# multimodallearning/convexAdam

Hardware: AMD Instinct MI355X
Metric: volume-pairs/sec (160x192x224 MIND convex+Adam(80it)) (higher is better)
Workload: dtype f32

## Files before the change

### convexadam_amd/csrc/certify.hip

```cpp
#include <hip/hip_runtime.h>
#include <stdlib.h>

#include "cvx_common.h"

namespace cvx {

#define CERT_CLO ((float)((1.0 - 1.0 / 65536.0) / 729.0))
#define CERT_CHI ((float)((1.0 + 1.0 / 65536.0) / 729.0))
#define CERT_TINY 1.0e-40f
__device__ __forceinline__ float cert_lower(float s) { return fmaxf(__builtin_fmaf(s, CERT_CLO, -CERT_TINY), 0.0f); }
__device__ __forceinline__ float cert_upper(float s) { return __builtin_fmaf(s, CERT_CHI, fminf(s, CERT_TINY)); }

__device__ __forceinline__ unsigned ordered_bits(float v) {
    unsigned b = __float_as_uint(v);
    b = (b & 0x80000000u) ? ~b : (b | 0x80000000u);
    if (v != v) b = 0u;
    return b;
}
__device__ __forceinline__ float from_ordered_bits(unsigned b) { return __uint_as_float((b & 0x80000000u) ? (b & 0x7fffffffu) : ~b); }

struct CertRec { unsigned x, box; int kp; float bound, slo, uc, ub, ua; };

struct CertProb {
    const float* ssdu; const float* fix; const float* mov; const float* tail;
    unsigned long long* key; unsigned* sec;
    int* idx0; int* idxA; int* idxB;
    float* smin;
    unsigned* list; int* counts;
    unsigned long long* work; unsigned work_cap;
    struct CertRec* rec;
    float* u;
    int64_t* argmin_out;
};
struct CertGeo { int C, h, w, d, hw, n, K, ntail; long long tail_from; };
struct CertArgs { CertProb p[2]; CertGeo g; const float* mesh; float coef; int pass; };

template <bool WAVE>
__device__ __forceinline__ void cert_sync() {
    if (WAVE) { __builtin_amdgcn_fence(__ATOMIC_RELEASE, "wavefront"); __builtin_amdgcn_s_waitcnt(0xC07F); __builtin_amdgcn_wave_barrier(); __builtin_amdgcn_fence(__ATOMIC_ACQUIRE, "wavefront"); }
    else __syncthreads();
}
template <bool WAVE>
__device__ float cert_exact_entry_t(const CertGeo& G, const CertProb& P, int k, int xlin, float* sm, int lane) {
    const int n = G.n, nn = n * n, h = G.h, w = G.w, d = G.d, hw = G.hw;
    const int iH = k % n, iW = (k / n) % n, iD = k / nn;
    const int x = xlin % d, y = (xlin / d) % w, z = xlin / (d * w);
    const size_t v = (size_t)h * w * d;
    for (int t = lane; t < 125; t += 64) {
        const int a = t / 25 - 2, b = (t / 5) % 5 - 2, c = t % 5 - 2;
        const int pz = z + a, py = y + b, px = x + c;
        float val = 0.0f;
        if (pz >= 0 && pz < h && py >= 0 && py < w && px >= 0 && px < d) {
            const long long flat = (((long long)pz * nn + iW * n + iD) * w + py) * d + px;
            if (G.ntail > 0 && flat >= G.tail_from) val = P.tail[iH * 32 + (int)(flat - G.tail_from)];
            else {
                const int mz = pz + iH - hw, my = py + iW - hw, mx = px + iD - hw;
                const bool inb = mz >= 0 && mz < h && my >= 0 && my < w && mx >= 0 && mx < d;
                const float* fp = P.fix + ((size_t)pz * w + py) * d + px;
                const float* mp = P.mov + ((size_t)(inb ? mz : 0) * w + (inb ? my : 0)) * d + (inb ? mx : 0);
                float a0 = 0.0f, a1 = 0.0f;
                for (int c0 = 0; c0 < G.C; c0 += 16) {
                    float fv[16], mv[16];
#pragma unroll
                    for (int i = 0; i < 16; ++i) {
                        const bool on = c0 + i < G.C;
                        fv[i] = on ? fp[(size_t)(c0 + i) * v] : 0.0f;
                        mv[i] = (on && inb) ? mp[(size_t)(c0 + i) * v] : 0.0f;
                    }
#pragma unroll
                    for (int i = 0; i < 16; ++i) {
                        if (c0 + i < G.C) {
                            const float df = fv[i] - mv[i];
                            a0 += df * df;
                        }
                    }
                    if (c0 + 16 <= G.C) { a1 += a0; a0 = 0.0f; }
                }
                val = G.C >= 16 ? a0 + a1 : a0;
            }
        }
        sm[t] = val;
    }
    cert_sync<WAVE>();
    if (lane < 27) {
        const int a = lane / 9 - 1, b = (lane / 3) % 3 - 1, c = lane % 3 - 1;
        const int pz = z + a, py = y + b, px = x + c;
        float s = 0.0f;
        const bool in = pz >= 0 && pz < h && py >= 0 && py < w && px >= 0 && px < d;
        if (in) {
            for (int aa = -1; aa <= 1; ++aa)
                for (int bb = -1; bb <= 1; ++bb)
                    for (int cc = -1; cc <= 1; ++cc) {
                        const int qz = pz + aa, qy = py + bb, qx = px + cc;
                        if (qz >= 0 && qz < h && qy >= 0 && qy < w && qx >= 0 && qx < d) s += sm[((a + aa + 2) * 5 + (b + bb + 2)) * 5 + (c + cc + 2)];
                    }
            s = div_exact<27>(s);
        }
        sm[128 + lane] = in ? s : -1.0f;
    }
    cert_sync<WAVE>();
    float s = 0.0f;
    for (int t = 0; t < 27; ++t) {
        const float b = sm[128 + t];
        if (b >= 0.0f || b != b) s += b;
    }
    cert_sync<WAVE>();
    return div_exact<27>(s);
}

__device__ float cert_exact_entry(const CertGeo& G, const CertProb& P, int k, int xlin, float* sm, int lane) { return cert_exact_entry_t<false>(G, P, k, xlin, sm, lane); }
__device__ float cert_exact_entry_wave(const CertGeo& G, const CertProb& P, int k, int xlin, float* sm, int lane) { return cert_exact_entry_t<true>(G, P, k, xlin, sm, lane); }

__global__ __launch_bounds__(256) void k_cert_plain_stream(CertArgs A, int kslice, int vec4) {
    const CertProb& P = A.p[blockIdx.z];
    const size_t v = (size_t)A.g.h * A.g.w * A.g.d;
    const int K = A.g.K;
    const size_t x0 = ((size_t)blockIdx.x * blockDim.x + threadIdx.x) * 4;
    const int k0 = blockIdx.y * kslice, k1 = min(k0 + kslice, K);
    if (x0 >= v) return;
    const int nv = (int)min((size_t)4, v - x0);
    const float INF = __uint_as_float(0x7f800000u);
    float best[4], second[4];
    int bi[4];
    bool tiny[4] = {false, false, false, false};
    const float* p = P.ssdu + (size_t)k0 * v + x0;
    auto load4 = [&](const float* q, float (&c4)[4]) {
        if (vec4) { const float4 t = *reinterpret_cast<const float4*>(q); c4[0] = t.x; c4[1] = t.y; c4[2] = t.z; c4[3] = t.w; }
        else {
#pragma unroll
            for (int j = 0; j < 4; ++j) c4[j] = j < nv ? q[j] : 0.0f;
        }
    };
    {
        float c4[4];
        load4(p, c4);
#pragma unroll
        for (int j = 0; j < 4; ++j) { best[j] = c4[j]; bi[j] = k0; second[j] = INF; tiny[j] = (c4[j] > 0.0f) & (c4[j] < 1.0e-36f); }
        p += v;
    }
#pragma unroll 8
    for (int k = k0 + 1; k < k1; ++k, p += v) {
        float c4[4];
        load4(p, c4);
#pragma unroll
        for (int j = 0; j < 4; ++j) {
            const float c = c4[j];
            tiny[j] = tiny[j] | ((c > 0.0f) & (c < 1.0e-36f));
            const bool lt = argmin_better(c, best[j]);
            second[j] = fminf(second[j], lt ? best[j] : c);
            best[j] = lt ? c : best[j];
            bi[j] = lt ? k : bi[j];
        }
    }
#pragma unroll
    for (int j = 0; j < 4; ++j) {
        if (j >= nv) continue;
        const unsigned long long mine = pack_min_key(best[j], (unsigned)bi[j]);
        const unsigned long long old = atomicMin(&P.key[x0 + j], mine);
        unsigned cand = second[j] == INF ? 0xffffffffu : ordered_bits(second[j]);
        if (old != ~0ull) {
            const unsigned loser = (unsigned)((old < mine ? mine : old) >> 32);
            cand = loser < cand ? loser : cand;
        }
        if (tiny[j]) cand = 0u;
        if (cand != 0xffffffffu) atomicMin(&P.sec[x0 + j], cand);
    }
}

__global__ __launch_bounds__(256) void k_cert_plain_finalize(CertArgs A) {
    const CertProb& P = A.p[blockIdx.y];
    const size_t v = (size_t)A.g.h * A.g.w * A.g.d;
    const size_t x = (size_t)blockIdx.x * blockDim.x + threadIdx.x;
    if (x >= v) return;
    const unsigned long long key = P.key[x];
    const unsigned b1 = (unsigned)(key >> 32), b2 = P.sec[x];
    const int k1 = (int)(unsigned)(key & 0xffffffffull);
    const float s1 = b1 == 0u ? __uint_as_float(0x7fc00000u) : from_ordered_bits(b1);
    P.smin[x] = s1;
    P.idx0[x] = k1;
    if (P.argmin_out) P.argmin_out[x] = k1;
    bool certain = b1 == 0u || b2 == 0xffffffffu;
    if (!certain && b2 != 0u) certain = s1 == 0.0f || cert_lower(from_ordered_bits(b2)) > cert_upper(s1);
    if (!certain) P.list[atomicAdd(&P.counts[0], 1)] = (unsigned)x;
}

__global__ __launch_bounds__(64) void k_cert_plain_resolve(CertArgs A) {
    __shared__ float sm[160];
    const CertProb& P = A.p[blockIdx.y];
    const size_t v = (size_t)A.g.h * A.g.w * A.g.d;
    const int K = A.g.K, lane = threadIdx.x;
    const int cnt = P.counts[0];
    for (int e = blockIdx.x; e < cnt; e += gridDim.x) {
        const unsigned x = P.list[e];
        const float* col = P.ssdu + x;
        const float U = cert_upper(P.smin[x]);
        unsigned long long bestkey = ~0ull;
        for (int kb = 0; kb < K; kb += 1024) {
            float s[16];
#pragma unroll
            for (int i = 0; i < 16; ++i) { const int k = kb + 64 * i + lane; s[i] = k < K ? col[(size_t)k * v] : __uint_as_float(0x7f800000u); }
#pragma unroll
            for (int i = 0; i < 16; ++i) {
                const unsigned long long mz = __ballot(s[i] == 0.0f);
                if (mz) {
                    const unsigned long long key = pack_min_key(0.0f, (unsigned)(kb + 64 * i + __ffsll((long long)mz) - 1));
                    bestkey = key < bestkey ? key : bestkey;
                }
                const bool mine = s[i] != 0.0f && cert_lower(s[i]) <= U;
                const unsigned long long m = __ballot(mine);
                if (m) {
                    const int nm = __popcll(m);
                    int base = 0;
                    if (lane == 0) base = atomicAdd(&P.counts[8], nm);
                    base = __shfl(base, 0);
                    const int slot = base + __popcll(m & ((1ull << lane) - 1ull));
                    if (mine && (unsigned)slot < P.work_cap) P.work[slot] = ((unsigned long long)x << 32) | (unsigned)(kb + 64 * i + lane);
                    unsigned long long rest = __ballot(mine && (unsigned)slot >= P.work_cap);
                    while (rest) {
                        const int l = __ffsll((long long)rest) - 1;
                        rest &= rest - 1;
                        const int kk = kb + 64 * i + l;
                        const float ex = cert_exact_entry(A.g, P, kk, (int)x, sm, lane);
                        const unsigned long long key = pack_min_key(ex, (unsigned)kk);
                        bestkey = key < bestkey ? key : bestkey;
                    }
                }
            }
        }
        if (lane == 0) P.key[x] = bestkey;
    }
}
__global__ __launch_bounds__(256) void k_cert_plain_eval(CertArgs A) {
    __shared__ float smem[4][160];
    const CertProb& P = A.p[blockIdx.y];
    const int lane = threadIdx.x & 63, wv = threadIdx.x >> 6;
    const int n = min(P.counts[8], (int)P.work_cap);
    for (int e = blockIdx.x * 4 + wv; e < n; e += gridDim.x * 4) {
        const unsigned long long it = P.work[e];
        const unsigned x = (unsigned)(it >> 32);
        const int kk = (int)(unsigned)(it & 0xffffffffull);
        const float ex = cert_exact_entry_wave(A.g, P, kk, (int)x, smem[wv], lane);
        if (lane == 0) atomicMin(&P.key[x], pack_min_key(ex, (unsigned)kk));
    }
}
__global__ __launch_bounds__(256) void k_cert_plain_commit(CertArgs A) {
    const CertProb& P = A.p[blockIdx.y];
    const int cnt = P.counts[0];
    for (int e = blockIdx.x * blockDim.x + threadIdx.x; e < cnt; e += gridDim.x * blockDim.x) {
        const unsigned x = P.list[e];
        const int kw = (int)(unsigned)(P.key[x] & 0xffffffffull);
        P.idx0[x] = kw;
        if (P.argmin_out) P.argmin_out[x] = kw;
    }
}

struct CertMesh {
    const float* ax;
    int n; float rn;
    __device__ __forceinline__ void split(int k, int& ic, int& ib, int& ia) const {
        const int q = (int)(((float)k + 0.5f) * rn);
        ic = k - q * n;
        ia = (int)(((float)q + 0.5f) * rn);
        ib = q - ia * n;
    }
};
__device__ __forceinline__ CertMesh cert_mesh_load(float* lds96, const float* __restrict__ mesh, int K, int n) {
    const int t = threadIdx.x;
    if (t < n) { lds96[t] = mesh[t]; lds96[32 + t] = mesh[K + t * n]; lds96[64 + t] = mesh[2 * K + t * n * n]; }
    __syncthreads();
    return CertMesh{lds96, n, 1.0f / (float)n};
}

__device__ __forceinline__ void cert_smooth_winner(const int* __restrict__ idx, const CertMesh& M, int h, int w, int d, size_t i,
                                                   float& o0, float& o1, float& o2) {
    const int x = (int)(i % d), y = (int)((i / d) % w), z = (int)(i / ((size_t)d * w));
    float s0 = 0.f, s1 = 0.f, s2 = 0.f;
#pragma unroll
    for (int a = -1; a <= 1; ++a) {
        const int za = z + a;
        const bool zok = za >= 0 && za < h;
        const int zc = zok ? za : z;
        int kk[9];
        bool ok[9];
#pragma unroll
        for (int b = -1; b <= 1; ++b)
#pragma unroll
            for (int c = -1; c <= 1; ++c) {
                const int yb = y + b, xc = x + c;
                const bool in = zok && yb >= 0 && yb < w && xc >= 0 && xc < d;
                const int t = (b + 1) * 3 + (c + 1);
                ok[t] = in;
                kk[t] = idx[((size_t)zc * w + (in ? yb : y)) * d + (in ? xc : x)];
            }
        float m0[9], m1[9], m2[9];
#pragma unroll
        for (int t = 0; t < 9; ++t) {
            int ic, ib, ia;
            M.split(kk[t], ic, ib, ia);
            m0[t] = M.ax[ic]; m1[t] = M.ax[32 + ib]; m2[t] = M.ax[64 + ia];
        }
#pragma unroll
        for (int t = 0; t < 9; ++t) {
            s0 += ok[t] ? m0[t] : 0.0f;
            s1 += ok[t] ? m1[t] : 0.0f;
            s2 += ok[t] ? m2[t] : 0.0f;
        }
    }
    o0 = fdiv(s0, 27.0f);
    o1 = fdiv(s1, 27.0f);
    o2 = fdiv(s2, 27.0f);
}

__device__ __forceinline__ float cert_pen(const CertMesh& M, int k, float uc, float ub, float ua, float coef) {
    int ic, ib, ia;
    M.split(k, ic, ib, ia);
    const float e0 = M.ax[ic] - uc, e1 = M.ax[32 + ib] - ub, e2 = M.ax[64 + ia] - ua;
    float q = e0 * e0;
    q += e1 * e1;
    q += e2 * e2;
    return coef * q;
}

struct CertBox {
    float uc, ub, ua, slo, bound;
    int c_lo, c_hi, b_lo, b_hi, a_lo, a_hi;
    long long vol;
    bool degenerate;
};
__device__ __forceinline__ CertBox cert_box(const CertMesh& M, float uc, float ub, float ua, float coef, int K, int n, int kp,
                                            float ssdu_kp, float smin_u, const float* __restrict__ col, size_t v, int refine_above) {
    CertBox c;
    c.uc = uc; c.ub = ub; c.ua = ua;
    c.slo = cert_lower(smin_u);
    c.bound = cert_upper(ssdu_kp) + cert_pen(M, kp, uc, ub, ua, coef);
    const float hwf = (float)((n - 1) / 2);
    auto close_box = [&]() {
        const float qmax = fdiv((c.bound - c.slo) + fabsf(c.bound) * 2.384185791015625e-07f, coef) * 1.00001f;
        const float R = fsqrt(fmaxf(qmax, 0.0f)) * 1.00001f + 1.0e-4f;
        c.c_lo = max((int)ceilf(c.uc - R + hwf), 0); c.c_hi = min((int)floorf(c.uc + R + hwf), n - 1);
        c.b_lo = max((int)ceilf(c.ub - R + hwf), 0); c.b_hi = min((int)floorf(c.ub + R + hwf), n - 1);
        c.a_lo = max((int)ceilf(c.ua - R + hwf), 0); c.a_hi = min((int)floorf(c.ua + R + hwf), n - 1);
        c.vol = (long long)max(c.c_hi - c.c_lo + 1, 0) * max(c.b_hi - c.b_lo + 1, 0) * max(c.a_hi - c.a_lo + 1, 0);
        c.degenerate = !(coef > 0.0f) || !(R == R) || c.vol <= 0;
    };
    close_box();
    if (!c.degenerate && c.vol > refine_above && uc == uc && ub == ub && ua == ua) {
        const int kn = (min(max((int)rintf(ua + hwf), 0), n - 1) * n + min(max((int)rintf(ub + hwf), 0), n - 1)) * n + min(max((int)rintf(uc + hwf), 0), n - 1);
        if (kn != kp) {
            const float near_hi = cert_upper(col[(size_t)kn * v]) + cert_pen(M, kn, uc, ub, ua, coef);
            if (near_hi < c.bound) { c.bound = near_hi; close_box(); }
        }
    }
    if (c.degenerate) { c.c_lo = c.b_lo = c.a_lo = 0; c.c_hi = c.b_hi = c.a_hi = n - 1; c.vol = (long long)n * n * n; }
    return c;
}

__global__ __launch_bounds__(64) void k_cert_voxel(CertArgs A, int refine) {
    const CertProb& P = A.p[blockIdx.y];
    const int h = A.g.h, w = A.g.w, d = A.g.d, K = A.g.K, n = A.g.n;
    const size_t v = (size_t)h * w * d;
    const size_t x = (size_t)blockIdx.x * blockDim.x + threadIdx.x;
    __shared__ float axes[96];
    const CertMesh M = cert_mesh_load(axes, A.mesh, K, n);
    if (x >= v) return;
    const int* prev = A.pass == 1 ? P.idx0 : ((A.pass & 1) ? P.idxB : P.idxA);
    int* next = (A.pass & 1) ? P.idxA : P.idxB;
    const int kp = prev[x];
    const float s_kp = P.ssdu[(size_t)kp * v + x];
    const float sm_x = P.smin[x];
    float uc, ub, ua;
    cert_smooth_winner(prev, M, h, w, d, x, uc, ub, ua);
    P.u[x] = uc; P.u[v + x] = ub; P.u[2 * v + x] = ua;
    if (sm_x != sm_x) { next[x] = P.idx0[x]; return; }
    const CertBox c = cert_box(M, uc, ub, ua, A.coef, K, n, kp, s_kp, sm_x, P.ssdu + x, v, refine);
    constexpr int NB = 8;
    const unsigned boxpack = (unsigned)c.c_lo | ((unsigned)c.c_hi << 5) | ((unsigned)c.b_lo << 10) | ((unsigned)c.b_hi << 15) | ((unsigned)c.a_lo << 20) | ((unsigned)c.a_hi << 25) | (c.degenerate ? 1u << 30 : 0u);
    const CertRec rec = {(unsigned)x, boxpack, kp, c.bound, c.slo, c.uc, c.ub, c.ua};
    if (c.vol > NB) { P.rec[atomicAdd(&P.counts[A.pass], 1)] = rec; return; }
    int kk[NB];
    float pen[NB], val[NB];
    bool need[NB];
    {
        int ic = c.c_lo, ib = c.b_lo, ia = c.a_lo;
#pragma unroll
        for (int j = 0; j < NB; ++j) {
            const bool in = j < (int)c.vol;
            kk[j] = (ia * n + ib) * n + ic;
            pen[j] = cert_pen(M, kk[j], c.uc, c.ub, c.ua, A.coef);
            need[j] = in && !(c.slo + pen[j] > c.bound);
            if (j + 1 < (int)c.vol) {
                if (++ic > c.c_hi) { ic = c.c_lo; if (++ib > c.b_hi) { ib = c.b_lo; ++ia; } }
            }
        }
    }
#pragma unroll
    for (int j = 0; j < NB; ++j) val[j] = need[j] ? P.ssdu[(size_t)kk[j] * v + x] : 0.0f;
    float lo1 = 0.f, lo2 = 0.f, U = __uint_as_float(0x7f800000u);
    int k1 = -1, cnt = 0;
#pragma unroll
    for (int j = 0; j < NB; ++j) {
        if (!need[j]) continue;
        const float lo = cert_lower(val[j]) + pen[j], hi = cert_upper(val[j]) + pen[j];
        U = fminf(U, hi);
        if (cnt == 0) { lo1 = lo; k1 = kk[j]; }
        else if (lo < lo1) { lo2 = lo1; lo1 = lo; k1 = kk[j]; }
        else if (cnt == 1 || lo < lo2) lo2 = lo;
        ++cnt;
    }
    if (cnt == 0) { next[x] = kp; return; }
    if (cnt == 1 || lo2 > U) { next[x] = k1; return; }
    P.rec[atomicAdd(&P.counts[A.pass], 1)] = rec;
}

__global__ __launch_bounds__(256) void k_cert_wave(CertArgs A) {
    __shared__ float smem[4][160];
    __shared__ float axes[96];
    const CertProb& P = A.p[blockIdx.y];
    const int h = A.g.h, w = A.g.w, d = A.g.d, K = A.g.K, n = A.g.n;
    const size_t v = (size_t)h * w * d;
    const int lane = threadIdx.x & 63, wv = threadIdx.x >> 6;
    float* sm = smem[wv];
    const CertMesh M = cert_mesh_load(axes, A.mesh, K, n);
    int* next = (A.pass & 1) ? P.idxA : P.idxB;
    const int cnt = P.counts[A.pass];
    const float INF = __uint_as_float(0x7f800000u);
    for (int e = blockIdx.x * 4 + wv; e < cnt; e += gridDim.x * 4) {
        const CertRec r = P.rec[e];
        const size_t x = r.x;
        const int kp = r.kp;
        const float* col = P.ssdu + x;
        CertBox c;
        c.uc = r.uc; c.ub = r.ub; c.ua = r.ua; c.slo = r.slo; c.bound = r.bound;
        c.c_lo = r.box & 31; c.c_hi = (r.box >> 5) & 31; c.b_lo = (r.box >> 10) & 31; c.b_hi = (r.box >> 15) & 31; c.a_lo = (r.box >> 20) & 31; c.a_hi = (r.box >> 25) & 31;
        c.degenerate = ((r.box >> 30) & 1u) != 0;
        c.vol = (long long)(c.c_hi - c.c_lo + 1) * (c.b_hi - c.b_lo + 1) * (c.a_hi - c.a_lo + 1);
        const int nc = c.c_hi - c.c_lo + 1, nb = c.b_hi - c.b_lo + 1, ncb = nc * nb;
        const float rc = 1.0f / (float)nc, rab = 1.0f / (float)ncb;
        unsigned long long key = ~0ull;
        float lo2 = INF, U = INF;
        constexpr int NL = 12;
        for (long long i0 = 0; i0 < c.vol; i0 += 64 * NL) {
            int kk[NL];
            float pen[NL], val[NL];
            bool need[NL];
#pragma unroll
            for (int j = 0; j < NL; ++j) {
                need[j] = false; kk[j] = 0; pen[j] = 0.0f;
                if (i0 + 64 * j < c.vol) {
                    const int i = (int)i0 + lane + 64 * j;
                    need[j] = i < (int)c.vol;
                    const int ii = need[j] ? i : 0;
                    const int qa = (int)(((float)ii + 0.5f) * rab), ra = ii - qa * ncb;
                    const int qb = (int)(((float)ra + 0.5f) * rc);
                    const int ic = c.c_lo + ra - qb * nc, ib = c.b_lo + qb, ia = c.a_lo + qa;
                    kk[j] = (ia * n + ib) * n + ic;
                    pen[j] = cert_pen(M, kk[j], c.uc, c.ub, c.ua, A.coef);
                    need[j] = need[j] && (c.degenerate || !(c.slo + pen[j] > c.bound));
                }
            }
#pragma unroll
            for (int j = 0; j < NL; ++j) val[j] = need[j] ? col[(size_t)kk[j] * v] : 0.0f;
#pragma unroll
            for (int j = 0; j < NL; ++j) {
                if (!need[j]) continue;
                const float lo = cert_lower(val[j]) + pen[j], hi = cert_upper(val[j]) + pen[j];
                U = fminf(U, hi);
                const unsigned long long kx = pack_min_key(lo, (unsigned)kk[j]);
                if (kx < key) { if (key != ~0ull) lo2 = fminf(lo2, from_ordered_bits((unsigned)(key >> 32))); key = kx; }
                else lo2 = fminf(lo2, lo);
            }
        }
        unsigned long long gkey = key;
        for (int o = 32; o > 0; o >>= 1) { const unsigned long long t = __shfl_xor(gkey, o); gkey = t < gkey ? t : gkey; }
        float mine2 = key == gkey ? lo2 : fminf(lo2, key != ~0ull ? from_ordered_bits((unsigned)(key >> 32)) : INF);
        for (int o = 32; o > 0; o >>= 1) { mine2 = fminf(mine2, __shfl_xor(mine2, o)); U = fminf(U, __shfl_xor(U, o)); }
        if (gkey == ~0ull) { if (lane == 0) next[x] = kp; continue; }
        if (mine2 > U) { if (lane == 0) next[x] = (int)(unsigned)(gkey & 0xffffffffull); continue; }
        if (lane == 0) atomicAdd(&P.counts[7], 1);
        unsigned long long bestkey = ~0ull;
        for (long long i0 = 0; i0 < c.vol; i0 += 64 * NL) {
            int kk[NL];
            float pen[NL], val[NL];
            bool need[NL];
#pragma unroll
            for (int j = 0; j < NL; ++j) {
                need[j] = false; kk[j] = 0; pen[j] = 0.0f;
                if (i0 + 64 * j < c.vol) {
                    const int i = (int)i0 + lane + 64 * j;
                    need[j] = i < (int)c.vol;
                    const int ii = need[j] ? i : 0;
                    const int qa = (int)(((float)ii + 0.5f) * rab), ra = ii - qa * ncb;
                    const int qb = (int)(((float)ra + 0.5f) * rc);
                    kk[j] = ((c.a_lo + qa) * n + c.b_lo + qb) * n + c.c_lo + ra - qb * nc;
                    pen[j] = cert_pen(M, kk[j], c.uc, c.ub, c.ua, A.coef);
                    need[j] = need[j] && (c.degenerate || !(c.slo + pen[j] > c.bound));
                }
            }
#pragma unroll
            for (int j = 0; j < NL; ++j) val[j] = need[j] ? col[(size_t)kk[j] * v] : 0.0f;
#pragma unroll
            for (int j = 0; j < NL; ++j) {
                if (!(i0 + 64 * j < c.vol)) continue;
                unsigned long long m = __ballot(need[j] && cert_lower(val[j]) + pen[j] <= U);
                while (m) {
                    const int l = __ffsll((long long)m) - 1;
                    m &= m - 1;
                    const int k2 = __shfl(kk[j], l);
                    const float sk = __shfl(val[j], l), pk = __shfl(pen[j], l);
                    const float ex = sk == 0.0f ? 0.0f : cert_exact_entry_wave(A.g, P, k2, (int)x, sm, lane);
                    const unsigned long long kx = pack_min_key(ex + pk, (unsigned)k2);
                    bestkey = kx < bestkey ? kx : bestkey;
                }
            }
        }
        if (lane == 0) next[x] = (int)(unsigned)(bestkey & 0xffffffffull);
    }
}

__global__ __launch_bounds__(256) void k_cert_gather(CertArgs A) {
    const CertProb& P = A.p[blockIdx.y];
    const size_t v = (size_t)A.g.h * A.g.w * A.g.d;
    const size_t i = (size_t)blockIdx.x * blockDim.x + threadIdx.x;
    __shared__ float axes[96];
    const CertMesh M = cert_mesh_load(axes, A.mesh, A.g.K, A.g.n);
    if (i >= v) return;
    const int* prev = A.pass == 1 ? P.idx0 : ((A.pass & 1) ? P.idxB : P.idxA);
    float o0, o1, o2;
    cert_smooth_winner(prev, M, A.g.h, A.g.w, A.g.d, i, o0, o1, o2);
    P.u[i] = o0; P.u[v + i] = o1; P.u[2 * v + i] = o2;
}

__global__ __launch_bounds__(256) void k_cert_arm(CertArgs A, int nprob) {
    const size_t v = (size_t)A.g.h * A.g.w * A.g.d;
    const size_t i = (size_t)blockIdx.x * blockDim.x + threadIdx.x;
    for (int q = 0; q < nprob; ++q) {
        if (i < v) { A.p[q].key[i] = ~0ull; A.p[q].sec[i] = 0xffffffffu; }
        if (i < 16) A.p[q].counts[i] = 0;
    }
}

void launch_corr_tail_compact(const float* fix, const float* mov, int C, int h, int w, int d, int hw, int sad, float* tail, hipStream_t s);

static size_t cert_work_cap(size_t v) { return 4 * v + 65536; }
struct CertCarve { unsigned long long* key; unsigned* sec; int* idx0; int* idxA; int* idxB; float* smin; unsigned* list; CertRec* rec; int* counts; float* tail; unsigned long long* work; unsigned work_cap; };
static CertCarve cert_layout(Carver& cv, int h, int w, int d, int hw, bool plain) {
    const size_t v = (size_t)h * w * d;
    const int n = 2 * hw + 1;
    CertCarve c{};
    c.key = cv.take<unsigned long long>(v);
    c.sec = cv.take<unsigned>(v);
    c.idx0 = cv.take<int>(v);
    c.smin = cv.take<float>(v);
    c.list = cv.take<unsigned>(v);
    c.counts = cv.take<int>(16);
    c.work_cap = (unsigned)cert_work_cap(v);
    c.work = cv.take<unsigned long long>(c.work_cap);
    c.tail = cv.take<float>((size_t)32 * n);
    if (!plain) {
        c.idxA = cv.take<int>(v); c.idxB = cv.take<int>(v);
        c.rec = cv.take<CertRec>(v);
    }
    return c;
}
size_t corr_certify_workspace_bytes(int, int h, int w, int d, int hw, bool plain) { Carver m; cert_layout(m, h, w, d, hw, plain); return ws_query(m); }
static CertGeo cert_geo(int C, int h, int w, int d, int hw) {
    CertGeo g;
    g.C = C; g.h = h; g.w = w; g.d = d; g.hw = hw; g.n = 2 * hw + 1; g.K = g.n * g.n * g.n;
    const long long ncols = (long long)h * g.n * g.n * w * d;
    g.tail_from = (ncols / 32) * 32;
    g.ntail = (int)(ncols - g.tail_from);
    return g;
}
static CertProb cert_prob(const float* ssdu, const float* fix, const float* mov, const CertCarve& c, float* u, int64_t* argmin_out) {
    return CertProb{ssdu, fix, mov, c.tail, c.key, c.sec, c.idx0, c.idxA, c.idxB, c.smin, c.list, c.counts, c.work, c.work_cap, c.rec, u, argmin_out};
}

static void cert_arm(CertArgs& A, int nprob, hipStream_t s) {
    const CertGeo& g = A.g;
    const size_t v = (size_t)g.h * g.w * g.d;
    hipLaunchKernelGGL(k_cert_arm, dim3((unsigned)cdiv64((int64_t)(v > 16 ? v : 16), 256)), dim3(256), 0, s, A, nprob);
    for (int q = 0; q < nprob; ++q)
        if (g.ntail > 0) launch_corr_tail_compact(A.p[q].fix, A.p[q].mov, g.C, g.h, g.w, g.d, g.hw, 0, const_cast<float*>(A.p[q].tail), s);
}
static void cert_stream(CertArgs A, int q0, int nq, hipStream_t s) {
    const CertGeo& g = A.g;
    const size_t v = (size_t)g.h * g.w * g.d;
    const int K = g.K;
    if (q0) { A.p[0] = A.p[q0]; }
    bool vec4 = v % 4 == 0;
    for (int q = 0; q < nq; ++q) vec4 = vec4 && (reinterpret_cast<uintptr_t>(A.p[q].ssdu) & 15) == 0;
    const int xb = (int)cdiv64((int64_t)cdiv64((int64_t)v, 4), 256);
    int nslices = cdiv(512, xb);
    if (nslices > K) nslices = K;
    if (nslices < 1) nslices = 1;
    const int kslice = cdiv(K, nslices);
    nslices = cdiv(K, kslice);
    hipLaunchKernelGGL(k_cert_plain_stream, dim3(xb, nslices, nq), dim3(256), 0, s, A, kslice, vec4 ? 1 : 0);
}
static int cert_finish(CertArgs& A, int nprob, hipStream_t s) {
    const size_t v = (size_t)A.g.h * A.g.w * A.g.d;
    hipLaunchKernelGGL(k_cert_plain_finalize, dim3((unsigned)cdiv64((int64_t)v, 256), nprob), dim3(256), 0, s, A);
    hipLaunchKernelGGL(k_cert_plain_resolve, dim3(256, nprob), dim3(64), 0, s, A);
    hipLaunchKernelGGL(k_cert_plain_eval, dim3(256, nprob), dim3(256), 0, s, A);
    hipLaunchKernelGGL(k_cert_plain_commit, dim3(8, nprob), dim3(256), 0, s, A);
    return check_last("certified argmin");
}
static int cert_plain(CertArgs& A, int nprob, bool arm, hipStream_t s) {
    if (arm) cert_arm(A, nprob, s);
    cert_stream(A, 0, nprob, s);
    return cert_finish(A, nprob, s);
}

int corr_certified_argmin(const float* ssdu, const float* fix, const float* mov, int C, int h, int w, int d, int hw, int64_t* argmin,
                          void* workspace, size_t workspace_bytes, hipStream_t s) {
    if (workspace_bytes < corr_certify_workspace_bytes(C, h, w, d, hw, true)) return fail(CVX_ERR_WORKSPACE, "certified argmin: workspace too small");
    Carver cv(workspace);
    const CertCarve c = cert_layout(cv, h, w, d, hw, true);
    CertArgs A{};
    A.g = cert_geo(C, h, w, d, hw);
    A.p[0] = cert_prob(ssdu, fix, mov, c, nullptr, argmin);
    A.p[1] = A.p[0];
    return cert_plain(A, 1, true, s);
}

int coupled_convex_cert_impl(const float* ssduA, const float* fixA, const float* movA, float* outA, void* wsA, const float* ssduB, const float* fixB,
                             const float* movB, float* outB, void* wsB, const float* mesh, int C, int h, int w, int d, int hw, size_t workspace_bytes,
                             hipStream_t s, int stage) {
    if (workspace_bytes < corr_certify_workspace_bytes(C, h, w, d, hw, false)) return fail(CVX_ERR_WORKSPACE, "certified coupled convex: workspace too small");
    const int nprob = ssduB ? 2 : 1;
    CertArgs A{};
    A.g = cert_geo(C, h, w, d, hw);
    A.mesh = mesh;
    Carver cva(wsA), cvb(wsB);
    const CertCarve ca = cert_layout(cva, h, w, d, hw, false);
    A.p[0] = cert_prob(ssduA, fixA, movA, ca, outA, nullptr);
    A.p[1] = A.p[0];
    if (ssduB) { const CertCarve cb = cert_layout(cvb, h, w, d, hw, false); A.p[1] = cert_prob(ssduB, fixB, movB, cb, outB, nullptr); }
    if (stage == 1) { cert_arm(A, nprob, s); return check_last("certified argmin"); }
    if (stage == 2) { cert_stream(A, 0, 1, s); return check_last("certified argmin"); }
    if (stage == 3) { if (nprob > 1) cert_stream(A, 1, 1, s); return check_last("certified argmin"); }
    if (stage == 4) return cert_finish(A, nprob, s);
    if (stage == 0) { const int rc = cert_plain(A, nprob, true, s); if (rc) return rc; }
    const size_t v = (size_t)h * w * d;
    const int refine = options().prune_refine != 0 ? 8 : 0x7fffffff;
    static const float coeffs[6] = {0.003f, 0.01f, 0.03f, 0.1f, 0.3f, 1.0f};
    for (int it = 0; it < 6; ++it) {
        A.coef = coeffs[it]; A.pass = it + 1;
        hipLaunchKernelGGL(k_cert_voxel, dim3((unsigned)cdiv64((int64_t)v, 64), nprob), dim3(64), 0, s, A, refine);
        hipLaunchKernelGGL(k_cert_wave, dim3(512, nprob), dim3(256), 0, s, A);
    }
    if (getenv("CVX_CERT_TRACE")) {
        for (int q = 0; q < nprob; ++q) {
            int cnt[8];
            (void)hipStreamSynchronize(s);
            (void)hipMemcpy(cnt, A.p[q].counts, sizeof(cnt), hipMemcpyDeviceToHost);
            fprintf(stderr, "cert trace: problem %d: plain flagged %d; listed per coupled pass %d %d %d %d %d %d, %d of them evaluated exactly (of %zu voxels)\n", q, cnt[0], cnt[1], cnt[2], cnt[3], cnt[4], cnt[5], cnt[6], cnt[7], v);
        }
    }
    A.pass = 7;
    hipLaunchKernelGGL(k_cert_gather, dim3((unsigned)cdiv64((int64_t)v, 256), nprob), dim3(256), 0, s, A);
    return check_last("certified coupled convex");
}

}
```

### convexadam_amd/csrc/cvx_common.h

```cpp
#pragma once
#include <hip/hip_runtime.h>
#include <stdint.h>
#include <stdio.h>
#include <stdarg.h>

#include <mutex>

#include "convexadam_hip.h"

namespace cvx {

void set_error(const char* fmt, ...);
int fail(int code, const char* fmt, ...);
int check_last(const char* what);

#define CVX_REQUIRE(cond, ...)                                      \
    do {                                                            \
        if (!(cond)) return ::cvx::fail(CVX_ERR_INVALID_ARG, __VA_ARGS__); \
    } while (0)

static inline hipStream_t as_stream(void* s) { return reinterpret_cast<hipStream_t>(s); }
static inline size_t align_up(size_t v, size_t a) { return (v + a - 1) / a * a; }
static inline int cdiv(int a, int b) { return (a + b - 1) / b; }
static inline int64_t cdiv64(int64_t a, int64_t b) { return (a + b - 1) / b; }

template <typename KernelT>
static inline void ensure_dynamic_lds(KernelT kernel, size_t bytes, size_t& granted) {
    static std::mutex mu;
    std::lock_guard<std::mutex> lock(mu);
    if (bytes > granted) {
        (void)hipFuncSetAttribute(reinterpret_cast<const void*>(kernel), hipFuncAttributeMaxDynamicSharedMemorySize, (int)bytes);
        (void)hipGetLastError();
        granted = bytes;
    }
}

struct Carver {
    char* base = nullptr;
    size_t used = 0;
    Carver() = default;
    explicit Carver(void* p) : base(static_cast<char*>(p)) {}
    size_t take_bytes(size_t bytes) { const size_t off = align_up(used, 256); used = off + bytes; return off; }
    template <typename T> T* take(size_t count) { const size_t off = take_bytes(count * sizeof(T)); return base ? reinterpret_cast<T*>(base + off) : nullptr; }
};
static inline size_t ws_query(const Carver& m) { return m.used ? m.used + 256 : 0; }

#define CVX_OPTIONS(X) \
    X(mind_tiled,          "CVX_MIND_TILED",            0)   \
    X(mind_overlap,        "CVX_MIND_OVERLAP",          0)   \
    X(mm_tx,               "CVX_MM_TX",                 0)   \
    X(mm_slots,            "CVX_MM_SLOTS",            512)   \
    X(box_tiled,           "CVX_BOX_TILED",             0)   \
    X(no_prune,            "CVX_NO_PRUNE",              0)   \
    X(corr_unfused,        "CVX_CORR_UNFUSED",          0)   \
    X(corr_fused_all,      "CVX_CORR_FUSED_ALL",        0)   \
    X(prune_stream_above,  "CVX_PRUNE_STREAM_ABOVE",   -1)   \
    X(cf_census,           "CVX_CF_CENSUS",             0)   \
    X(cf_prio,             "CVX_CF_PRIO",             136)   \
    X(warp_flat,           "CVX_WARP_FLAT",             0)   \
    X(box_yt,              "CVX_BOX_YT",                8)   \
    X(box_wg_target,       "CVX_BOX_WG_TARGET",         0)   \
    X(box_xsplit,          "CVX_BOX_XSPLIT",           -1)   \
    X(box_cpt,             "CVX_BOX_CPT",               4)   \
    X(box_uneven,          "CVX_BOX_UNEVEN",          200)   \
    X(box_adam_role,       "CVX_BOX_ADAM_ROLE",         0)   \
    X(box_dpp,             "CVX_BOX_DPP",               0)   \
    X(box_pk,              "CVX_BOX_PK",                0)   \
    X(box_prio,            "CVX_BOX_PRIO",              0)   \
    X(label_pow_block,     "CVX_LABEL_POW_BLOCK",      32)   \
    X(census_ptr,          nullptr,                     0)   \
    X(mind_mean_threads,   "CVX_MIND_MEAN_THREADS",     0)   \
    X(edt_sequential,      "CVX_EDT_SEQUENTIAL",        0)   \
    X(warp_octant,         "CVX_WARP_OCTANT",           4)   \
    X(box_fwd_tile,        "CVX_BOX_FWD_TILE",         -1)   \
    X(box_bwd_tile,        "CVX_BOX_BWD_TILE",         -1)   \
    X(box_walk,            "CVX_BOX_WALK",              1)   \
    X(corr_dual,           "CVX_CORR_DUAL",             0)   \
    X(prune_refine,        "CVX_PRUNE_REFINE",          1)   \
    X(mind_records,        "CVX_MIND_RECORDS",          1)   \
    X(resize_up2,          "CVX_RESIZE_UP2",            1)   \
    X(mind_blocked,        "CVX_MIND_BLOCKED",          1)   \
    X(corr_cert,           "CVX_CORR_CERT",             1)   \
    X(cc_debug,            "CVX_CC_DEBUG",              0)   \
    X(ic_fused,            "CVX_IC_FUSED",              0)   \
    X(mind_single,         "CVX_MIND_SINGLE",           0)   \
    X(ms_zlen,             "CVX_MS_ZLEN",               0)   \
    X(cf_map,              "CVX_CF_MAP",                1)   \
    X(cert_unfused,        "CVX_CERT_UNFUSED",          0)   \
    X(fbox_tile,           "CVX_FBOX_TILE",             0)   \
    X(box_tile_sync,       "CVX_BOX_TILE_SYNC",         0)   \
    X(box_prediv,          "CVX_BOX_PREDIV",            1)   \
    X(tile_census_ptr,     nullptr,                     0)   \
    X(adam_wt,             "CVX_ADAM_WT",               1)
#define X(name, env, dflt) long long name;
struct Options { CVX_OPTIONS(X) };
#undef X
Options& options();
const unsigned* adam_sqrt_table();
class ContextScope {
public:
    explicit ContextScope(const cvx_context* c);
    ~ContextScope();
    ContextScope(const ContextScope&) = delete;
    ContextScope& operator=(const ContextScope&) = delete;
private:
    void* prev_;
    bool active_;
};

#ifdef CVX_RACE_JITTER
__device__ __forceinline__ void cvx_jitter() {
    unsigned t = (unsigned)__builtin_amdgcn_s_memtime();
    t ^= (unsigned)__builtin_amdgcn_s_getreg((4 << 0) | (0 << 6) | (31 << 11)) * 2654435761u;
    t ^= t >> 13; t *= 0x9E3779B1u; t ^= t >> 15;
    const int n = (int)(t & 15);
    for (int i = 0; i < n; ++i) __builtin_amdgcn_s_sleep(1);
}
__device__ __forceinline__ void cvx_barrier() { cvx_jitter(); __syncthreads(); cvx_jitter(); }
#else
__device__ __forceinline__ void cvx_barrier() { __syncthreads(); }
#endif

__device__ __forceinline__ int clampi(int v, int lo, int hi) { return v < lo ? lo : (v > hi ? hi : v); }

__device__ __forceinline__ float fdiv(float a, float b) { return __fdiv_rn(a, b); }
__device__ __forceinline__ float fsqrt(float a) { return sqrtf(a); }

__device__ __forceinline__ float cvx_expf(float d) {
    const float R_LN2f = 1.442695040888963407359924681001892137426645954152985934135449406931f;
    const float L2Uf = 0.693145751953125f, L2Lf = 1.428606765330187045e-06f;
    const float qf = rintf(d * R_LN2f);
    const int q = (int)qf;
    float s = __builtin_fmaf(qf, -L2Uf, d);
    s = __builtin_fmaf(qf, -L2Lf, s);
    float u = 0.000198527617612853646278381f;
    u = __builtin_fmaf(u, s, 0.00139304355252534151077271f);
    u = __builtin_fmaf(u, s, 0.00833336077630519866943359f);
    u = __builtin_fmaf(u, s, 0.0416664853692054748535156f);
    u = __builtin_fmaf(u, s, 0.166666671633720397949219f);
    u = __builtin_fmaf(u, s, 0.5f);
    u = 1.0f + __builtin_fmaf(s * s, u, s);
    u = __builtin_ldexpf(u, q);
    if (d < -104.0f) u = 0.0f;
    if (d > 100.0f) u = __int_as_float(0x7f800000);
    return u;
}

struct ExpTable { const unsigned char* tbl; unsigned first, count; };
ExpTable mind_exp_table();

typedef float f32x4 __attribute__((ext_vector_type(4)));
typedef __attribute__((address_space(3))) f32x4 lds_f32x4;
__device__ __forceinline__ f32x4 lds_load4(const float* p) { return *(const volatile lds_f32x4*)p; }
__device__ __forceinline__ void lds_store4(float* p, f32x4 v) { *(volatile lds_f32x4*)p = v; }

typedef int i32x4 __attribute__((ext_vector_type(4)));
typedef unsigned u32x4 __attribute__((ext_vector_type(4)));
__device__ __forceinline__ float4 buffer_load16(__amdgpu_buffer_rsrc_t rsrc, unsigned lane_off, unsigned uni_off) {
    const i32x4 v = __builtin_bit_cast(i32x4, __builtin_amdgcn_raw_buffer_load_b128(rsrc, (int)lane_off, (int)uni_off, 0));
    return make_float4(__int_as_float(v.x), __int_as_float(v.y), __int_as_float(v.z), __int_as_float(v.w));
}

template <bool WT>
__device__ __forceinline__ void buffer_store16(__amdgpu_buffer_rsrc_t rsrc, unsigned lane_off, unsigned uni_off, float4 v) {
    __builtin_amdgcn_raw_buffer_store_b128(__builtin_bit_cast(u32x4, v), rsrc, (int)lane_off, (int)uni_off, WT ? 16 : 0);
}
template <bool WT>
__device__ __forceinline__ void buffer_store4(__amdgpu_buffer_rsrc_t rsrc, unsigned lane_off, unsigned uni_off, float v) {
    __builtin_amdgcn_raw_buffer_store_b32(__float_as_uint(v), rsrc, (int)lane_off, (int)uni_off, WT ? 16 : 0);
}
__device__ __forceinline__ void global_store16_wt(float* p, float4 v) {
    asm volatile("global_store_dwordx4 %0, %1, off sc1\n\ts_nop 1" : : "v"(p), "v"(__builtin_bit_cast(f32x4, v)) : "memory");
}

typedef float f32x2 __attribute__((ext_vector_type(2)));
typedef __attribute__((address_space(3))) f32x2 lds_f32x2;
__device__ __forceinline__ f32x2 lds_load2(const float* p) { return *(const volatile lds_f32x2*)p; }
__device__ __forceinline__ void lds_store2(float* p, f32x2 v) { *(volatile lds_f32x2*)p = v; }

template <int D>
__device__ __forceinline__ float div_exact(float x) {
    static_assert(D == 8 || D == 27 || D == 64 || D == 125 || D == 343, "divisor not verified");
    constexpr float r = 1.0f / (float)D;
    const float q = x * r;
    const float e = __builtin_fmaf(-(float)D, q, x);
    return __builtin_fmaf(e, r, q);
}
template <int D>
__device__ __forceinline__ float div_exact_inf(float x) { return __builtin_isinf(x) ? x : div_exact<D>(x); }

struct ConstDiv { float d, r; int ok; };
constexpr float kConstDivLo = 0x1p-76f, kConstDivHi = 0x1p76f;
ConstDiv const_div_ieee(float d);
ConstDiv const_div_make(float d);
ConstDiv const_div(float d);
ConstDiv const_div_if_proven(float d);
bool const_div_enumerate(float d, float r);
void const_div_prove(const float* ds, int n, int budget);
__device__ __forceinline__ float div_const_seq(float x, const ConstDiv& cd) {
    const float q = x * cd.r;
    const float e = __builtin_fmaf(-cd.d, q, x);
    return __builtin_fmaf(e, cd.r, q);
}
__device__ __forceinline__ bool div_const_inside(float x) { const float a = __builtin_fabsf(x); return a >= kConstDivLo && a <= kConstDivHi; }
__device__ __forceinline__ bool div_const_inside_root(float x) { return x <= kConstDivHi; }
__device__ __forceinline__ bool wave_all(bool inside) { return __builtin_amdgcn_ballot_w64(!inside) == 0; }
__device__ __forceinline__ float div_const(float x, const ConstDiv& cd) {
    if (cd.ok && wave_all(div_const_inside(x))) return div_const_seq(x, cd);
    return fdiv(x, cd.d);
}

template <int N>
__device__ __forceinline__ float cascade_seq(const float (&v)[N]) {
    static_assert(N < 256, "two cascade levels");
    float a0 = 0.f, a1 = 0.f;
    int i = 0;
#pragma unroll
    for (; i + 16 <= N; i += 16) {
#pragma unroll
        for (int j = 0; j < 16; ++j) a0 += v[i + j];
        a1 += a0;
        a0 = 0.f;
    }
#pragma unroll
    for (; i < N; ++i) a0 += v[i];
    a0 += a1;
    return a0;
}
template <int N>
__device__ __forceinline__ float outer_sum_ilp(const float (&v)[N]) {
    static_assert(N / 4 < 16, "single cascade level inside the interleaved sums");
    float p[4] = {0.f, 0.f, 0.f, 0.f};
#pragma unroll
    for (int i = 0; i < N / 4; ++i)
#pragma unroll
        for (int k = 0; k < 4; ++k) p[k] += v[4 * i + k];
#pragma unroll
    for (int i = (N / 4) * 4; i < N; ++i) p[0] += v[i];
    p[0] += p[1];
    p[0] += p[2];
    p[0] += p[3];
    return p[0];
}

__device__ __forceinline__ unsigned long long pack_min_key(float v, unsigned idx) {
    unsigned b = __float_as_uint(v);
// ... 228 lines not shown
```

Measured before the change: 154.3.

## Chunk certified resolve across blocks and pair exact evaluations per wave

```diff
diff --git a/convexadam_amd/csrc/certify.hip b/convexadam_amd/csrc/certify.hip
--- a/convexadam_amd/csrc/certify.hip
+++ b/convexadam_amd/csrc/certify.hip
@@ -20,6 +20,8 @@
 __device__ __forceinline__ float from_ordered_bits(unsigned b) { return __uint_as_float((b & 0x80000000u) ? (b & 0x7fffffffu) : ~b); }
 
 struct CertRec { unsigned x, box; int kp; float bound, slo, uc, ub, ua; };
+
+#define CERT_QUEUE 64
 
 struct CertProb {
     const float* ssdu; const float* fix; const float* mov; const float* tail;
@@ -108,6 +110,100 @@
     return div_exact<27>(s);
 }
 
+__device__ void cert_exact_pair_wave(const CertGeo& G, const CertProb& P, int k0, int k1, int xlin, float* sm, int lane, float& ex0, float& ex1) {
+    const int n = G.n, nn = n * n, h = G.h, w = G.w, d = G.d, hw = G.hw;
+    const int x = xlin % d, y = (xlin / d) % w, z = xlin / (d * w);
+    const size_t v = (size_t)h * w * d;
+    const unsigned v32 = (unsigned)v;
+    unsigned fo[4], mo[4];
+    bool chan[4], inb[4];
+    float val[4], a0[4], a1[4];
+    int slot[4];
+#pragma unroll
+    for (int u = 0; u < 4; ++u) {
+        const int T = lane + 64 * u, cand = T >= 125 ? 1 : 0, t = T - 125 * cand;
+        const int k = cand ? k1 : k0;
+        const int iH = k % n, iW = (k / n) % n, iD = k / nn;
+        const int a = t / 25 - 2, b = (t / 5) % 5 - 2, c = t % 5 - 2;
+        const int pz = z + a, py = y + b, px = x + c;
+        const bool in = T < 250 && pz >= 0 && pz < h && py >= 0 && py < w && px >= 0 && px < d;
+        slot[u] = T < 250 ? cand * 160 + t : -1;
+        val[u] = 0.0f; a0[u] = 0.0f; a1[u] = 0.0f;
+        chan[u] = false; inb[u] = false; fo[u] = 0u; mo[u] = 0u;
+        if (in) {
+            const long long flat = (((long long)pz * nn + iW * n + iD) * w + py) * d + px;
+            if (G.ntail > 0 && flat >= G.tail_from) val[u] = P.tail[iH * 32 + (int)(flat - G.tail_from)];
+            else {
+                const int mz = pz + iH - hw, my = py + iW - hw, mx = px + iD - hw;
+                chan[u] = true;
+                inb[u] = mz >= 0 && mz < h && my >= 0 && my < w && mx >= 0 && mx < d;
+                fo[u] = (unsigned)((pz * w + py) * d + px);
+                mo[u] = (unsigned)(((inb[u] ? mz : 0) * w + (inb[u] ? my : 0)) * d + (inb[u] ? mx : 0));
+            }
+        }
+    }
+    const char* fbase = reinterpret_cast<const char*>(P.fix);
+    const char* mbase = reinterpret_cast<const char*>(P.mov);
+    for (int c0 = 0; c0 < G.C; c0 += 16) {
+        const int cend = min(c0 + 16, G.C);
+        for (int c1 = c0; c1 < cend; c1 += 6) {
+            float fv[4][6], mv[4][6];
+#pragma unroll
+            for (int u = 0; u < 4; ++u)
+#pragma unroll
+                for (int i = 0; i < 6; ++i) {
+                    const bool on = chan[u] && c1 + i < cend;
+                    fv[u][i] = on ? *reinterpret_cast<const float*>(fbase + (fo[u] + (unsigned)(c1 + i) * v32) * 4u) : 0.0f;
+                    mv[u][i] = (on && inb[u]) ? *reinterpret_cast<const float*>(mbase + (mo[u] + (unsigned)(c1 + i) * v32) * 4u) : 0.0f;
+                }
+#pragma unroll
+            for (int u = 0; u < 4; ++u)
+#pragma unroll
+                for (int i = 0; i < 6; ++i) {
+                    if (c1 + i < cend) {
+                        const float df = fv[u][i] - mv[u][i];
+                        a0[u] += df * df;
+                    }
+                }
+        }
+        if (c0 + 16 <= G.C) {
+#pragma unroll
+            for (int u = 0; u < 4; ++u) { a1[u] += a0[u]; a0[u] = 0.0f; }
+        }
+    }
+#pragma unroll
+    for (int u = 0; u < 4; ++u) {
+        if (chan[u]) val[u] = G.C >= 16 ? a0[u] + a1[u] : a0[u];
+        if (slot[u] >= 0) sm[slot[u]] = val[u];
+    }
+    cert_sync<true>();
+    float* smc = sm + (lane >> 5) * 160;
+    const int l = lane & 31;
+    if (l < 27) {
+        const int a = l / 9 - 1, b = (l / 3) % 3 - 1, c = l % 3 - 1;
+        const int pz = z + a, py = y + b, px = x + c;
+        const bool in = pz >= 0 && pz < h && py >= 0 && py < w && px >= 0 && px < d;
+        float tap[27];
+#pragma unroll
+        for (int q = 0; q < 27; ++q) tap[q] = smc[((a + q / 9 + 1) * 5 + (b + (q / 3) % 3 + 1)) * 5 + (c + q % 3 + 1)];
+        float s = 0.0f;
+#pragma unroll
+        for (int q = 0; q < 27; ++q) s += tap[q];
+        smc[128 + l] = in ? div_exact<27>(s) : -1.0f;
+    }
+    cert_sync<true>();
+    float box[27];
+#pragma unroll
+    for (int t = 0; t < 27; ++t) box[t] = smc[128 + t];
+    float s = 0.0f;
+#pragma unroll
+    for (int t = 0; t < 27; ++t) s += (box[t] >= 0.0f || box[t] != box[t]) ? box[t] : 0.0f;
+    cert_sync<true>();
+    s = div_exact<27>(s);
+    ex0 = __shfl(s, 0);
+    ex1 = __shfl(s, 32);
+}
+
 __device__ float cert_exact_entry(const CertGeo& G, const CertProb& P, int k, int xlin, float* sm, int lane) { return cert_exact_entry_t<false>(G, P, k, xlin, sm, lane); }
 __device__ float cert_exact_entry_wave(const CertGeo& G, const CertProb& P, int k, int xlin, float* sm, int lane) { return cert_exact_entry_t<true>(G, P, k, xlin, sm, lane); }
 
@@ -167,7 +263,7 @@
     }
 }
 
-__global__ __launch_bounds__(256) void k_cert_plain_finalize(CertArgs A) {
+__global__ __launch_bounds__(256) void k_cert_plain_finalize(CertArgs A, int reset_key) {
     const CertProb& P = A.p[blockIdx.y];
     const size_t v = (size_t)A.g.h * A.g.w * A.g.d;
     const size_t x = (size_t)blockIdx.x * blockDim.x + threadIdx.x;
@@ -181,21 +277,27 @@
     if (P.argmin_out) P.argmin_out[x] = k1;
     bool certain = b1 == 0u || b2 == 0xffffffffu;
     if (!certain && b2 != 0u) certain = s1 == 0.0f || cert_lower(from_ordered_bits(b2)) > cert_upper(s1);
-    if (!certain) P.list[atomicAdd(&P.counts[0], 1)] = (unsigned)x;
-}
-
+    if (!certain) {
+        P.list[atomicAdd(&P.counts[0], 1)] = (unsigned)x;
+        if (reset_key) P.key[x] = ~0ull;
+    }
+}
+
+template <bool CHUNK>
 __global__ __launch_bounds__(64) void k_cert_plain_resolve(CertArgs A) {
     __shared__ float sm[160];
     const CertProb& P = A.p[blockIdx.y];
     const size_t v = (size_t)A.g.h * A.g.w * A.g.d;
     const int K = A.g.K, lane = threadIdx.x;
     const int cnt = P.counts[0];
-    for (int e = blockIdx.x; e < cnt; e += gridDim.x) {
+    const int nch = CHUNK ? (K + 1023) / 1024 : 1;
+    for (long long t = blockIdx.x; t < (long long)cnt * nch; t += gridDim.x) {
+        const int e = (int)(t / nch), ch = (int)(t - (long long)e * nch);
         const unsigned x = P.list[e];
         const float* col = P.ssdu + x;
         const float U = cert_upper(P.smin[x]);
         unsigned long long bestkey = ~0ull;
-        for (int kb = 0; kb < K; kb += 1024) {
+        for (int kb = CHUNK ? ch * 1024 : 0; kb < (CHUNK ? min(K, (ch + 1) * 1024) : K); kb += 1024) {
             float s[16];
 #pragma unroll
             for (int i = 0; i < 16; ++i) { const int k = kb + 64 * i + lane; s[i] = k < K ? col[(size_t)k * v] : __uint_as_float(0x7f800000u); }
@@ -227,7 +329,8 @@
                 }
             }
         }
-        if (lane == 0) P.key[x] = bestkey;
+        if (CHUNK) { if (lane == 0 && bestkey != ~0ull) atomicMin(&P.key[x], bestkey); }
+        else if (lane == 0) P.key[x] = bestkey;
     }
 }
 __global__ __launch_bounds__(256) void k_cert_plain_eval(CertArgs A) {
@@ -412,8 +515,11 @@
     P.rec[atomicAdd(&P.counts[A.pass], 1)] = rec;
 }
 
-__global__ __launch_bounds__(256) void k_cert_wave(CertArgs A) {
-    __shared__ float smem[4][160];
+template <bool PAIR>
+__global__ __launch_bounds__(256, 2) void k_cert_wave(CertArgs A) {
+    __shared__ float smem[4][PAIR ? 320 : 160];
+    __shared__ int queue_k[PAIR ? 4 : 1][CERT_QUEUE];
+    __shared__ float queue_pen[PAIR ? 4 : 1][CERT_QUEUE];
     __shared__ float axes[96];
     const CertProb& P = A.p[blockIdx.y];
     const int h = A.g.h, w = A.g.w, d = A.g.d, K = A.g.K, n = A.g.n;
@@ -478,6 +584,7 @@
         if (mine2 > U) { if (lane == 0) next[x] = (int)(unsigned)(gkey & 0xffffffffull); continue; }
         if (lane == 0) atomicAdd(&P.counts[7], 1);
         unsigned long long bestkey = ~0ull;
+        int ncand = 0, nq = 0;
         for (long long i0 = 0; i0 < c.vol; i0 += 64 * NL) {
             int kk[NL];
             float pen[NL], val[NL];
@@ -502,18 +609,41 @@
             for (int j = 0; j < NL; ++j) {
                 if (!(i0 + 64 * j < c.vol)) continue;
                 unsigned long long m = __ballot(need[j] && cert_lower(val[j]) + pen[j] <= U);
+                ncand += __popcll(m);
                 while (m) {
                     const int l = __ffsll((long long)m) - 1;
                     m &= m - 1;
                     const int k2 = __shfl(kk[j], l);
                     const float sk = __shfl(val[j], l), pk = __shfl(pen[j], l);
+                    if (PAIR && sk != 0.0f && nq < CERT_QUEUE) {
+                        if (lane == 0) { queue_k[wv][nq] = k2; queue_pen[wv][nq] = pk; }
+                        ++nq;
+                        continue;
+                    }
                     const float ex = sk == 0.0f ? 0.0f : cert_exact_entry_wave(A.g, P, k2, (int)x, sm, lane);
                     const unsigned long long kx = pack_min_key(ex + pk, (unsigned)k2);
                     bestkey = kx < bestkey ? kx : bestkey;
                 }
             }
         }
-        if (lane == 0) next[x] = (int)(unsigned)(bestkey & 0xffffffffull);
+        if (PAIR && nq > 0) {
+            cert_sync<true>();
+            for (int q = 0; q + 1 < nq; q += 2) {
+                const int ka = queue_k[wv][q], kb = queue_k[wv][q + 1];
+                float ea, eb;
+                cert_exact_pair_wave(A.g, P, ka, kb, (int)x, sm, lane, ea, eb);
+                const unsigned long long xa = pack_min_key(ea + queue_pen[wv][q], (unsigned)ka), xb = pack_min_key(eb + queue_pen[wv][q + 1], (unsigned)kb);
+                bestkey = xa < bestkey ? xa : bestkey;
+                bestkey = xb < bestkey ? xb : bestkey;
+            }
+            if (nq & 1) {
+                const int ka = queue_k[wv][nq - 1];
+                const unsigned long long xa = pack_min_key(cert_exact_entry_wave(A.g, P, ka, (int)x, sm, lane) + queue_pen[wv][nq - 1], (unsigned)ka);
+                bestkey = xa < bestkey ? xa : bestkey;
+            }
+            cert_sync<true>();
+        }
+        if (lane == 0) { next[x] = (int)(unsigned)(bestkey & 0xffffffffull); atomicAdd(&P.counts[9], ncand); }
     }
 }
 
@@ -599,8 +729,10 @@
 }
 static int cert_finish(CertArgs& A, int nprob, hipStream_t s) {
     const size_t v = (size_t)A.g.h * A.g.w * A.g.d;
-    hipLaunchKernelGGL(k_cert_plain_finalize, dim3((unsigned)cdiv64((int64_t)v, 256), nprob), dim3(256), 0, s, A);
-    hipLaunchKernelGGL(k_cert_plain_resolve, dim3(256, nprob), dim3(64), 0, s, A);
+    const bool chunked = (options().cert_chunk & 1) != 0;
+    hipLaunchKernelGGL(k_cert_plain_finalize, dim3((unsigned)cdiv64((int64_t)v, 256), nprob), dim3(256), 0, s, A, chunked ? 1 : 0);
+    if (chunked) hipLaunchKernelGGL(k_cert_plain_resolve<true>, dim3(2048, nprob), dim3(64), 0, s, A);
+    else hipLaunchKernelGGL(k_cert_plain_resolve<false>, dim3(256, nprob), dim3(64), 0, s, A);
     hipLaunchKernelGGL(k_cert_plain_eval, dim3(256, nprob), dim3(256), 0, s, A);
     hipLaunchKernelGGL(k_cert_plain_commit, dim3(8, nprob), dim3(256), 0, s, A);
     return check_last("certified argmin");
@@ -621,6 +753,30 @@
     A.p[0] = cert_prob(ssdu, fix, mov, c, nullptr, argmin);
     A.p[1] = A.p[0];
     return cert_plain(A, 1, true, s);
+}
+
+static void cert_trace_boxes(const CertArgs& A, int nprob, hipStream_t s) {
+    for (int q = 0; q < nprob; ++q) {
+        int cnt = 0, exact = 0, ncand = 0;
+        (void)hipStreamSynchronize(s);
+        (void)hipMemcpy(&cnt, A.p[q].counts + A.pass, sizeof(int), hipMemcpyDeviceToHost);
+        (void)hipMemcpy(&exact, A.p[q].counts + 7, sizeof(int), hipMemcpyDeviceToHost);
+        (void)hipMemcpy(&ncand, A.p[q].counts + 9, sizeof(int), hipMemcpyDeviceToHost);
+        CertRec* rec = (CertRec*)malloc(sizeof(CertRec) * (size_t)(cnt > 0 ? cnt : 1));
+        if (!rec) return;
+        (void)hipMemcpy(rec, A.p[q].rec, sizeof(CertRec) * (size_t)cnt, hipMemcpyDeviceToHost);
+        long long hist[9] = {0}, entries = 0;
+        for (int e = 0; e < cnt; ++e) {
+            const unsigned b = rec[e].box;
+            const long long vol = (long long)(((b >> 5) & 31) - (b & 31) + 1) * (((b >> 15) & 31) - ((b >> 10) & 31) + 1) * (((b >> 25) & 31) - ((b >> 20) & 31) + 1);
+            const long long nch = (vol + 768 - 1) / 768;
+            hist[vol <= 64 ? 0 : (nch > 7 ? 8 : nch)]++;
+            entries += vol;
+        }
+        fprintf(stderr, "cert trace: problem %d pass %d: %d listed, %lld box entries; boxes of <= 64 entries: %lld, 65..768: %lld, chunks 2..7: %lld %lld %lld %lld %lld %lld, more: %lld; exact decisions so far: %d with %d candidates\n",
+                q, A.pass, cnt, entries, hist[0], hist[1], hist[2], hist[3], hist[4], hist[5], hist[6], hist[7], hist[8], exact, ncand);
+        free(rec);
+    }
 }
 
 int coupled_convex_cert_impl(const float* ssduA, const float* fixA, const float* movA, float* outA, void* wsA, const float* ssduB, const float* fixB,
@@ -644,12 +800,16 @@
     const size_t v = (size_t)h * w * d;
     const int refine = options().prune_refine != 0 ? 8 : 0x7fffffff;
     static const float coeffs[6] = {0.003f, 0.01f, 0.03f, 0.1f, 0.3f, 1.0f};
+    const bool pair = (options().cert_chunk & 2) != 0 && (unsigned long long)C * v * 4ull < (1ull << 32);
+    const char* trace = getenv("CVX_CERT_TRACE");
     for (int it = 0; it < 6; ++it) {
         A.coef = coeffs[it]; A.pass = it + 1;
         hipLaunchKernelGGL(k_cert_voxel, dim3((unsigned)cdiv64((int64_t)v, 64), nprob), dim3(64), 0, s, A, refine);
-        hipLaunchKernelGGL(k_cert_wave, dim3(512, nprob), dim3(256), 0, s, A);
-    }
-    if (getenv("CVX_CERT_TRACE")) {
+        if (pair) hipLaunchKernelGGL(k_cert_wave<true>, dim3(512, nprob), dim3(256), 0, s, A);
+        else hipLaunchKernelGGL(k_cert_wave<false>, dim3(512, nprob), dim3(256), 0, s, A);
+        if (trace && atoi(trace) >= 2) cert_trace_boxes(A, nprob, s);
+    }
+    if (trace) {
         for (int q = 0; q < nprob; ++q) {
             int cnt[8];
             (void)hipStreamSynchronize(s);
diff --git a/convexadam_amd/csrc/cvx_common.h b/convexadam_amd/csrc/cvx_common.h
--- a/convexadam_amd/csrc/cvx_common.h
+++ b/convexadam_amd/csrc/cvx_common.h
@@ -91,7 +91,8 @@
     X(box_tile_sync,       "CVX_BOX_TILE_SYNC",         0)   \
     X(box_prediv,          "CVX_BOX_PREDIV",            1)   \
     X(tile_census_ptr,     nullptr,                     0)   \
-    X(adam_wt,             "CVX_ADAM_WT",               1)
+    X(adam_wt,             "CVX_ADAM_WT",               1)   \
+    X(cert_chunk,          "CVX_CERT_CHUNK",            3)
 #define X(name, env, dflt) long long name;
 struct Options { CVX_OPTIONS(X) };
 #undef X
```

New measurement: 154.7 (median of 4 runs). No clear change (+0.3%).
